# hkust-vgd/scanobjectnn

Measured on NVIDIA H100. Metric: point-clouds/sec (B=32, N=2048, 15-class), higher is better.
Workload: dtype f32

## Files before the change

### scanobjectnn_b200/csrc/tc_mlp.cu

```cuda
#include <float.h>
#include <stdlib.h>

#include <algorithm>
#include <atomic>
#include <type_traits>

#include "common.cuh"
#include "mlp_internal.cuh"
#include "ring_gemm.cuh"
#include "tc_common.cuh"

namespace psa {

using namespace tc;

constexpr int kMaxTcLayers = 2;


struct TcArgs {
    long long groups;
    int K;
    int n, m;
    const float* xyz;
    const float* new_xyz;
    const float* uf;
    const int* idx;
    float* out;
    const float* w1c;
    const float* w1x;
    const float* s1;
    const float* t1;
    int C1, relu1;
    int nl;
    const uint8_t* image[kMaxTcLayers];
    const float* s[kMaxTcLayers];
    const float* t[kMaxTcLayers];
    int relu[kMaxTcLayers];
    int Kd[kMaxTcLayers], Ntot[kMaxTcLayers];
    int stream_last;
    int joint;
    int pool_chunks;
    unsigned int* tile_counter;
    int np;
    unsigned int* ovf;
    const unsigned int* run_if;
    const unsigned int* wflag[kMaxTcLayers];
    const float* colscale[kMaxTcLayers];
};

template <int NP, int S>
__device__ __forceinline__ void put_a(uint32_t (&A)[NP][S][4], int s, int r, float x0, float x1, uint32_t& ovf) {
    uint32_t p[NP];
    split_pair<NP>(x0, x1, p, ovf);
#pragma unroll
    for (int i = 0; i < NP; ++i) A[i][s][r] = p[i];
}

__device__ __forceinline__ float warp_rowmax16(float lo, float hi) {
    float m = fmaxf(lo, hi);
    m = fmaxf(m, __shfl_xor_sync(0xffffffffu, m, 4));
    m = fmaxf(m, __shfl_xor_sync(0xffffffffu, m, 8));
    m = fmaxf(m, __shfl_xor_sync(0xffffffffu, m, 16));
    return m;
}
template <int H, int S>
__device__ __forceinline__ void colmax_halve(float (&v)[S], bool up) {
#pragma unroll
    for (int i = 0; i < H; ++i) {
        const float lo = v[i], hi = v[H + i];
        v[i] = fmaxf(up ? hi : lo, __shfl_xor_sync(0xffffffffu, up ? lo : hi, 2 * H));
    }
}
__device__ __forceinline__ float warp_rowsum16(float v) {
    v += __shfl_xor_sync(0xffffffffu, v, 4);
    v += __shfl_xor_sync(0xffffffffu, v, 8);
    v += __shfl_xor_sync(0xffffffffu, v, 16);
    return v;
}

__global__ void __launch_bounds__(256) tc_col_scale_kernel(int K, int N, const float* __restrict__ W, float* __restrict__ colscale,
                                                           unsigned int* __restrict__ trailer) {
    __shared__ float s_max[8][32];
    __shared__ int s_bad[8][32];
    const int n = blockIdx.x * 32 + threadIdx.x;
    float m = 0.f;
    bool bad = false;
    if (n < N)
        for (int k = threadIdx.y; k < K; k += 8) {
            const float w = __ldg(W + (size_t)k * N + n);
            bad = bad || !isfinite(w);
            m = fmaxf(m, fabsf(w));
        }
    s_max[threadIdx.y][threadIdx.x] = m;
    s_bad[threadIdx.y][threadIdx.x] = bad;
    __syncthreads();
    if (threadIdx.y != 0 || n >= N) return;
    for (int y = 1; y < 8; ++y) { m = fmaxf(m, s_max[y][threadIdx.x]); bad = bad || s_bad[y][threadIdx.x]; }
    int e = 0;
    if (!bad && m > 0.f) e = min(137 - (int)(__float_as_uint(m) >> 23), 64);
    colscale[n] = __int_as_float((127 - e) << 23);
    if (bad) atomicOr(trailer, 1u);
}

template <int NP>
__global__ void tc_prep_weights_kernel(int K, int Kp, int N, int Nt, const float* __restrict__ W, const float* __restrict__ colscale,
                                       uint8_t* __restrict__ image, const unsigned int* __restrict__ run_if) {
    if (run_if != nullptr && *run_if == 0u) return;
    const int KC = Kp / 64;
    const uint32_t bb = tc_block_bytes(Nt, NP), piece = (uint32_t)Nt * 128u;
    uint32_t unused = 0u;
    for (int e = blockIdx.x * blockDim.x + threadIdx.x; e < Kp * N; e += gridDim.x * blockDim.x) {
        const int n = e % N, k = e / N;
        float w = k < K ? __ldg(W + e) : 0.f;
        if (NP == 2) w *= pow2_rcp(__ldg(colscale + n));
        uint32_t pc[NP];
        split_pair<NP>(w, 0.f, pc, unused);
        uint8_t* blk = image + (size_t)((n / Nt) * KC + (k >> 6)) * bb;
        const uint32_t off = swz_off_bf16(n % Nt, k & 63, Nt);
#pragma unroll
        for (int i = 0; i < NP; ++i) *reinterpret_cast<uint16_t*>(blk + i * piece + off) = (uint16_t)(pc[i] & 0xffffu);
    }
}

constexpr int kSaNt = 64;
constexpr int kSaThreads = 256;
constexpr uint32_t kSmemBudget = 220u * 1024u;

struct TcSaLayout {
    uint32_t w[kMaxTcLayers];
    uint32_t ring[2];
    uint32_t ring_bytes;
    uint32_t vec, total;
};

__host__ __device__ inline TcSaLayout tc_sa_layout(const TcArgs& a) {
    TcSaLayout L;
    uint32_t off = 0;
#pragma unroll
    for (int l = 0; l < kMaxTcLayers; ++l) {
        L.w[l] = off;
        if (l < a.nl && !(a.stream_last && l == a.nl - 1)) off += (uint32_t)tc_image_bytes(a.Kd[l], a.Ntot[l], a.np);
    }
    L.ring_bytes = a.stream_last ? (uint32_t)(a.Kd[a.nl - 1] / 64) * tc_block_bytes(kSaNt, a.np) : 0u;
    L.ring[0] = off; off += L.ring_bytes;
    L.ring[1] = off; off += L.ring_bytes;
    L.vec = off;
    off += 7u * a.C1 * 4u;
#pragma unroll
    for (int l = 0; l < kMaxTcLayers; ++l) off += l < a.nl ? 2u * a.Ntot[l] * 4u : 0u;
    L.total = off;
    return L;
}

__host__ __device__ inline int sa_chunk(int K, bool joint) { return (joint ? 128 : 512) / K; }
__host__ __device__ inline uint32_t sa_carry_bytes(const TcArgs& a) { return a.joint ? 0u : 2u * a.Ntot[a.nl - 1] * 4u; }
__host__ __device__ inline uint32_t sa_red_bytes(int chunks) { return 8u * 64u * 4u * (uint32_t)chunks; }

__device__ __forceinline__ void sa_fill_ring(uint32_t q, const uint8_t* image, int ncl, const TcSaLayout& L, uint8_t* base, uint64_t* bars) {
    uint64_t* bar = &bars[q & 1];
    mbar_expect_tx(bar, L.ring_bytes);
    const uint8_t* src = image + (size_t)(q % (uint32_t)ncl) * L.ring_bytes;
    for (uint32_t o = 0; o < L.ring_bytes; o += 32768u) bulk_g2s(base + L.ring[q & 1] + o, src + o, min(32768u, L.ring_bytes - o), bar);
}

template <int NP, int KS, int NCH>
__device__ __forceinline__ void sa_mma_issue(float (&d)[NCH][32], const uint32_t (&A)[NP][8][4], uint32_t wb, uint32_t cstride) {
    constexpr uint32_t bb = tc_block_bytes(kSaNt, NP), piece = kSaNt * 128u;
    wg_fence();
#pragma unroll
    for (int tt = 0; tt < Split<NP>::kTerms; ++tt)
#pragma unroll
        for (int s = 0; s < KS; ++s)
#pragma unroll
            for (int c = 0; c < NCH; ++c)
                wg_mma_rs<NP>(d[c], A[Split<NP>::a(tt)][s][0], A[Split<NP>::a(tt)][s][1], A[Split<NP>::a(tt)][s][2], A[Split<NP>::a(tt)][s][3],
                              wg_desc(wb + (uint32_t)c * cstride + (uint32_t)(s >> 2) * bb + Split<NP>::w(tt) * piece + (uint32_t)(s & 3) * 32u),
                              (tt | s) ? 1u : 0u);
    wg_commit();
}
template <int NP, int KS, int NCH>
__device__ __forceinline__ void sa_mma(float (&d)[NCH][32], const uint32_t (&A)[NP][8][4], uint32_t wb, uint32_t cstride) {
    sa_mma_issue<NP, KS, NCH>(d, A, wb, cstride);
    wg_wait_all();
#pragma unroll
    for (int c = 0; c < NCH; ++c) wg_fence_acc(d[c]);
}

#ifdef PSA_SA_STAMPS
enum SaStamp { kSaTop, kSaInputs, kSaLayer1, kSaL2Issued, kSaL2Retired, kSaL2Epi, kSaPool1, kSaPool2, kSaNextA, kSaNextB, kSaChunk0 };
constexpr int kSaStampCtas = 264, kSaStampPasses = 64, kSaStampPhases = kSaChunk0 + 3 * 4;
__device__ long long g_sa_stamps[kSaStampCtas][2][kSaStampPasses][kSaStampPhases];
extern "C" PSA_API int psa_sa_stamps(long long* dst) {
    return cudaMemcpyFromSymbol(dst, g_sa_stamps, sizeof(g_sa_stamps)) == cudaSuccess ? 0 : 1;
}
extern "C" PSA_API int psa_sa_stamps_clear(void) {
    void* p = nullptr;
    if (cudaGetSymbolAddress(&p, g_sa_stamps) != cudaSuccess) return 1;
    return cudaMemset(p, 0, sizeof(g_sa_stamps)) == cudaSuccess ? 0 : 1;
}
#define SA_STAMP(p, k)                                                                                              \
    do {                                                                                                            \
        if ((threadIdx.x & 127) == 0 && blockIdx.x < kSaStampCtas && (p) < kSaStampPasses && (k) < kSaStampPhases) \
            g_sa_stamps[blockIdx.x][threadIdx.x >> 7][(p)][(k)] = clock64();                                        \
    } while (0)
#define SA_STAMP_AFTER(p, k, r)                                                                                     \
    do {                                                                                                            \
        if ((threadIdx.x & 127) == 0 && blockIdx.x < kSaStampCtas && (p) < kSaStampPasses) {                        \
            volatile long long* p_ = &g_sa_stamps[blockIdx.x][threadIdx.x >> 7][(p)][(k)];                          \
            *p_ = (long long)__float_as_uint(__fmul_rn((r), 0.f));                                                  \
            *p_ = clock64();                                                                                        \
        }                                                                                                           \
    } while (0)
#else
#define SA_STAMP(p, k) \
    do {               \
    } while (0)
#define SA_STAMP_AFTER(p, k, r) \
    do {                        \
    } while (0)
#endif

template <int NP, int C1, int NL, int N0>
__global__ void __launch_bounds__(kSaThreads, NP == 2 && C1 == 64 && (NL == 1 || N0 == 64) ? 2 : 1)
tc_sa_kernel(const __grid_constant__ TcArgs a) {
    static_assert((C1 == 64 || C1 == 128) && (NL == 1 || (NL == 2 && (N0 == 64 || N0 == 128))), "unsupported level shape");
    constexpr int last = NL - 1;
    constexpr int KSL = (NL == 2 ? N0 : C1) / 16;
    constexpr bool kDouble = !(C1 == 64 && (NL == 1 || N0 == 64));
    if (a.run_if != nullptr && *a.run_if == 0u) return;
    constexpr uint32_t bb = tc_block_bytes(kSaNt, NP);
    uint32_t ovf = 0u;
    bool ovf_seen = false;
    extern __shared__ uint8_t smem_raw[];
    __shared__ __align__(8) uint64_t s_rbar;
    __shared__ __align__(8) uint64_t s_wbar[2];
    __shared__ unsigned int s_claim[2];
    __shared__ int s_slots[2][2][16];
    __shared__ long long s_desc[2][2][8];

    const int tid = threadIdx.x, lane = tid & 31, warp = tid >> 5;
    const int g = lane >> 2, t = lane & 3;
    uint8_t* base = smem_raw + ((1024u - (smem_u32(smem_raw) & 1023u)) & 1023u);
    const TcSaLayout L = tc_sa_layout(a);

    float* vec = reinterpret_cast<float*>(base + L.vec);
    float* w1x = vec;
    float* w1c = vec + 3 * C1;
    float* t1 = vec + 6 * C1;
    float* sl0 = t1 + C1;
    float* tl0 = sl0 + a.Ntot[0];
    float* slL = NL == 2 ? tl0 + a.Ntot[0] : sl0;
    float* tlL = slL + a.Ntot[last];
    for (int i = tid; i < 3 * C1; i += kSaThreads) {
        const float sc = a.s1 ? __ldg(a.s1 + i % C1) : 1.f;
        w1x[i] = __ldg(a.w1x + i) * sc;
        w1c[i] = (a.w1c ? __ldg(a.w1c + i) : 0.f) * sc - (a.uf ? w1x[i] : 0.f);
    }
    for (int i = tid; i < C1; i += kSaThreads) t1[i] = __ldg(a.t1 + i);
#pragma unroll
    for (int l = 0; l < NL; ++l)
        for (int i = tid; i < a.Ntot[l]; i += kSaThreads) {
            (l == 0 ? sl0 : slL)[i] = (a.s[l] ? __ldg(a.s[l] + i) : 1.f) * (NP == 2 ? __ldg(a.colscale[l] + i) : 1.f);
            (l == 0 ? tl0 : tlL)[i] = __ldg(a.t[l] + i);
        }
    if (tid == 0) {
        mbar_init(&s_rbar, 1); mbar_init(&s_wbar[0], 1); mbar_init(&s_wbar[1], 1);
        fence_mbar_init();
    }
    __syncthreads();

    const int NCL = a.Ntot[last] / 64;
    uint32_t resident = 0;
#pragma unroll
    for (int l = 0; l < NL; ++l)
        if (!(a.stream_last && l == last)) resident += (uint32_t)tc_image_bytes(a.Kd[l], a.Ntot[l], NP);
    if (tid == 0) {
        if (resident) {
            mbar_expect_tx(&s_rbar, resident);
#pragma unroll
            for (int l = 0; l < NL; ++l) {
                if (a.stream_last && l == last) continue;
                const uint32_t bytes = (uint32_t)tc_image_bytes(a.Kd[l], a.Ntot[l], NP);
                for (uint32_t o = 0; o < bytes; o += 32768u) bulk_g2s(base + L.w[l] + o, a.image[l] + o, min(32768u, bytes - o), &s_rbar);
            }
        }
        if (a.stream_last) { sa_fill_ring(0, a.image[last], NCL, L, base, s_wbar); sa_fill_ring(1, a.image[last], NCL, L, base, s_wbar); }
    }
    if (resident) mbar_wait(&s_rbar, 0);

    const int K = a.K;
    const bool joint = a.joint;
    const int W = joint ? 8 : 4;
    const int C = sa_chunk(K, joint);
    const int unit = joint ? 0 : warp >> 2;
    const int ubar = 1 + unit, uthreads = 32 * W;
    const int ut = joint ? tid : tid & 127, uw0 = joint ? 0 : 4 * unit;
    const int wl = warp - uw0;
    const unsigned nchunks = (unsigned)((a.groups + C - 1) / C);
    float* carry = reinterpret_cast<float*>(base + L.total) + (size_t)unit * a.Ntot[last];
    const int NG = a.pool_chunks, rs = 64 * NG;
    float* red = reinterpret_cast<float*>(base + L.total + sa_carry_bytes(a)) + (size_t)warp * rs;

    auto fill_table = [&](unsigned ch, int b) {
        const long long g0 = (long long)ch * C;
        if (joint) {
            if (ut < C) s_slots[unit][b][ut] = g0 + ut < a.groups ? K / 16 : 0;
            return;
        }
        const long long r0 = g0 * K + wl * 128, rows = a.groups * K;
        int v[4];
#pragma unroll
        for (int q = 0; q < 4; ++q) v[q] = r0 + 32 * q + lane < rows ? __ldg(a.idx + r0 + 32 * q + lane) : 0;
        if (K == 32) {
#pragma unroll
            for (int q = 0; q < 4; ++q) {
                const unsigned d = __ballot_sync(0xffffffffu, v[q] != __shfl_sync(0xffffffffu, v[q], 0));
                const int nb = 4 * wl + q, Ln = d ? 32 - __clz(d) : 1;
                if (lane == 0) s_slots[unit][b][nb] = g0 + nb < a.groups ? (Ln + 15) >> 4 : 0;
            }
        } else {
#pragma unroll
            for (int h = 0; h < 2; ++h) {
                const int f = __shfl_sync(0xffffffffu, v[2 * h], 0);
                const unsigned lo = __ballot_sync(0xffffffffu, v[2 * h] != f), hi = __ballot_sync(0xffffffffu, v[2 * h + 1] != f);
                const int nb = 2 * wl + h, Ln = hi ? 64 - __clz(hi) : lo ? 32 - __clz(lo) : 1;
                if (lane == 0) s_slots[unit][b][nb] = g0 + nb < a.groups ? (Ln + 15) >> 4 : 0;
            }
        }
    };

    constexpr bool kAhead = NL == 2;
    constexpr bool kHoldU = NP == 2 && C1 == 128 && kAhead;
    constexpr int kUH = kHoldU ? C1 / 8 : 1;
    int incl = 0;
    int jn[2];
    long long gn = 0;
    bool carry_next = false;
    float cx = 0.f, cy = 0.f, cz = 0.f, px[2], py[2], pz[2];
    const float* urow[2];
    float2 uh[2][kUH];
    auto gather_a = [&](unsigned ch, int b, int p, int d) {
        if (p == 0) {
            incl = lane < C ? s_slots[unit][b][lane] : 0;
#pragma unroll
            for (int o = 1; o < 16; o <<= 1) {
                const int y = __shfl_up_sync(0xffffffffu, incl, o);
                if (lane >= o) incl += y;
            }
        }
        const int T = __shfl_sync(0xffffffffu, incl, C - 1);
        const int s = p * W + wl, ss = min(s, T - 1);
        const int nb = __popc(__ballot_sync(0xffffffffu, incl <= ss) & ((1u << C) - 1u));
        const int end = __shfl_sync(0xffffffffu, incl, nb), start = nb ? __shfl_sync(0xffffffffu, incl, nb - 1) : 0;
        gn = (long long)ch * C + nb;
        const int row = 16 * (ss - start) + g;
#pragma unroll
        for (int i = 0; i < 2; ++i) jn[i] = __ldg(a.idx + gn * K + row + 8 * i);
        const float* c = a.new_xyz + (size_t)gn * 3;
        cx = __ldg(c); cy = __ldg(c + 1); cz = __ldg(c + 2);
        carry_next = wl == 0 && s < T && s > start;
        if (lane == 0) {
            long long run = 0;
            if (s < T && (wl == 0 || s == start)) {
                const int pe = (p + 1) * W;
                run = gn << 8 | (long long)(min(end, pe) - s) | (s > start ? 16 : 0) | (end > pe ? 32 : 0);
            }
            s_desc[unit][d][wl] = run;
        }
    };
    auto gather_b = [&]() {
        const long long bi = gn / a.m;
#pragma unroll
        for (int i = 0; i < 2; ++i) {
            if (a.uf == nullptr) {
                const float* p = a.xyz + ((size_t)bi * a.n + jn[i]) * 3;
                px[i] = __ldg(p); py[i] = __ldg(p + 1); pz[i] = __ldg(p + 2);
            }
            urow[i] = a.uf ? a.uf + ((size_t)bi * a.n + jn[i]) * C1 : nullptr;
            if constexpr (kHoldU) {
                if (a.uf != nullptr) {
#pragma unroll
                    for (int q = 0; q < kUH; ++q) uh[i][q] = __ldg(reinterpret_cast<const float2*>(urow[i] + 8 * q + 2 * t));
                }
            }
        }
    };

    if (ut == 0) s_claim[unit] = atomicAdd(a.tile_counter, 1u);
    unit_bar_sync(ubar, uthreads);
    unsigned ch = s_claim[unit], claimed = 0;
    if (ch < nchunks) fill_table(ch, 0);
    unit_bar_sync(ubar, uthreads);
    int buf = 0, p = 0;
    if (kAhead && ch < nchunks) { gather_a(ch, 0, 0, 0); gather_b(); }
    uint32_t it = 0;
    for (; ch < nchunks; ++it) {
        if (p == 0 && ut == 0) s_claim[unit] = atomicAdd(a.tile_counter, 1u);
        SA_STAMP(it, kSaTop);
        if (!kAhead) { gather_a(ch, buf, p, it & 1); gather_b(); }
        SA_STAMP_AFTER(it, kSaInputs, a.uf == nullptr ? px[0] : kHoldU ? uh[0][0].x : __ldg(urow[0] + 2 * t));

        uint32_t A[NP][8][4];
        if (a.uf != nullptr) {
#pragma unroll
            for (int s = 0; s < C1 / 16; ++s) {
#pragma unroll
                for (int h = 0; h < 2; ++h) {
                    const int k = 16 * s + 8 * h + 2 * t;
                    const float2 cwx = *reinterpret_cast<const float2*>(w1c + k), cwy = *reinterpret_cast<const float2*>(w1c + C1 + k),
                                 cwz = *reinterpret_cast<const float2*>(w1c + 2 * C1 + k);
                    const float2 ct = ffma2_rn(make_float2(cz, cz), cwz, ffma2_rn(make_float2(cy, cy), cwy, fmul2_rn(make_float2(cx, cx), cwx)));
#pragma unroll
                    for (int i = 0; i < 2; ++i) {
                        float2 v;
                        if constexpr (kHoldU) v = uh[i][2 * s + h];
                        else v = __ldg(reinterpret_cast<const float2*>(urow[i] + k));
                        v = fadd2_rn(v, ct);
                        if (a.relu1) { v.x = fmaxf(v.x, 0.f); v.y = fmaxf(v.y, 0.f); }
                        put_a<NP, 8>(A, s, i + 2 * h, v.x, v.y, ovf);
                    }
                }
            }
        } else {
            float dx[2], dy[2], dz[2];
#pragma unroll
            for (int i = 0; i < 2; ++i) { dx[i] = px[i] - cx; dy[i] = py[i] - cy; dz[i] = pz[i] - cz; }
#pragma unroll
            for (int s = 0; s < C1 / 16; ++s) {
#pragma unroll
                for (int h = 0; h < 2; ++h) {
                    const int k = 16 * s + 8 * h + 2 * t;
                    const float2 sh = *reinterpret_cast<const float2*>(t1 + k);
                    const float2 wx = *reinterpret_cast<const float2*>(w1x + k), wy = *reinterpret_cast<const float2*>(w1x + C1 + k),
                                 wz = *reinterpret_cast<const float2*>(w1x + 2 * C1 + k);
#pragma unroll
                    for (int i = 0; i < 2; ++i) {
                        float2 v = sh;
                        if (a.w1c != nullptr) {
                            const float2 cwx = *reinterpret_cast<const float2*>(w1c + k), cwy = *reinterpret_cast<const float2*>(w1c + C1 + k),
                                         cwz = *reinterpret_cast<const float2*>(w1c + 2 * C1 + k);
                            v = ffma2_rn(make_float2(cz, cz), cwz, ffma2_rn(make_float2(cy, cy), cwy, ffma2_rn(make_float2(cx, cx), cwx, v)));
                        }
                        v = ffma2_rn(make_float2(dz[i], dz[i]), wz, ffma2_rn(make_float2(dy[i], dy[i]), wy, ffma2_rn(make_float2(dx[i], dx[i]), wx, v)));
                        if (a.relu1) { v.x = fmaxf(v.x, 0.f); v.y = fmaxf(v.y, 0.f); }
                        put_a<NP, 8>(A, s, i + 2 * h, v.x, v.y, ovf);
                    }
                }
            }
        }
        SA_STAMP(it, kSaLayer1);

        if constexpr (NL == 2) {
            constexpr int NCH = N0 / 64;
            float d[NCH][32];
            sa_mma_issue<NP, C1 / 16, NCH>(d, A, smem_u32(base + L.w[0]), (uint32_t)(C1 / 64) * bb);
            SA_STAMP(it, kSaL2Issued);
            wg_wait_all();
#pragma unroll
            for (int c = 0; c < NCH; ++c) wg_fence_acc(d[c]);
            SA_STAMP(it, kSaL2Retired);
#pragma unroll
            for (int c = 0; c < NCH; ++c) {
#pragma unroll
                for (int jj = 0; jj < 4; ++jj) {
#pragma unroll
                    for (int h = 0; h < 2; ++h) {
                        const int j = 2 * jj + h, col = c * 64 + 8 * j + 2 * t;
                        const float sc0 = sl0[col], sc1 = sl0[col + 1], sh0 = tl0[col], sh1 = tl0[col + 1];
#pragma unroll
                        for (int i = 0; i < 2; ++i) {
                            float v0 = fmaf(d[c][4 * j + 2 * i], sc0, sh0), v1 = fmaf(d[c][4 * j + 2 * i + 1], sc1, sh1);
                            if (a.relu[0]) { v0 = fmaxf(v0, 0.f); v1 = fmaxf(v1, 0.f); }
                            put_a<NP, 8>(A, c * 4 + jj, i + 2 * h, v0, v1, ovf);
                        }
                    }
                }
            }
            SA_STAMP(it, kSaL2Epi);
        }
        if constexpr (NP == 2) { ovf_seen = ovf_seen || f16x2_overflowed(ovf); ovf = 0u; }
        {
            const int N = a.Ntot[last];
            const bool carry_in = carry_next;
            const bool same = (p + 1) * W < __shfl_sync(0xffffffffu, incl, C - 1);
            const bool ahead = kAhead && (same || (p > 0 && claimed < nchunks));
            const bool after_pool = kAhead && !same && p == 0;
            auto issue = [&](float (&acc)[1][32], int nc) {
                uint32_t wb;
                if (a.stream_last) {
                    const uint32_t q = it * (uint32_t)NCL + (uint32_t)nc;
                    mbar_wait(&s_wbar[q & 1], (q >> 1) & 1u);
                    wb = smem_u32(base + L.ring[q & 1]);
                } else {
                    wb = smem_u32(base + L.w[last]) + (uint32_t)(nc * (KSL / 4)) * bb;
                }
                sa_mma_issue<NP, KSL, 1>(acc, A, wb, 0u);
                SA_STAMP(it, kSaChunk0 + 3 * nc);
            };
            auto epilogue = [&](float (&acc)[1][32], int nc) {
                wg_fence_acc(acc[0]);
                SA_STAMP(it, kSaChunk0 + 3 * nc + 1);
                auto rowmax = [&](int j) {
                    const int col = nc * 64 + 8 * j + 2 * t;
                    const float2 sc = *reinterpret_cast<const float2*>(slL + col), sh = *reinterpret_cast<const float2*>(tlL + col);
                    float lo0 = fmaf(acc[0][4 * j], sc.x, sh.x), hi0 = fmaf(acc[0][4 * j + 2], sc.x, sh.x);
                    float lo1 = fmaf(acc[0][4 * j + 1], sc.y, sh.y), hi1 = fmaf(acc[0][4 * j + 3], sc.y, sh.y);
                    if (a.relu[last]) { lo0 = fmaxf(lo0, 0.f); hi0 = fmaxf(hi0, 0.f); lo1 = fmaxf(lo1, 0.f); hi1 = fmaxf(hi1, 0.f); }
                    return make_float2(fmaxf(lo0, hi0), fmaxf(lo1, hi1));
                };
                float v[8];
                const bool up = (g >> 2) & 1;
#pragma unroll
                for (int j = 0; j < 4; ++j) {
                    const float2 lo = rowmax(j), hi = rowmax(j + 4);
                    v[2 * j] = fmaxf(up ? hi.x : lo.x, __shfl_xor_sync(0xffffffffu, up ? lo.x : hi.x, 16));
                    v[2 * j + 1] = fmaxf(up ? hi.y : lo.y, __shfl_xor_sync(0xffffffffu, up ? lo.y : hi.y, 16));
                }
                colmax_halve<4>(v, (g >> 1) & 1);
                colmax_halve<2>(v, g & 1);
                float2 m = make_float2(v[0], v[1]);
                const int x = 8 * g + 2 * t;
                float* dst = red + (nc % NG) * 64 + x;
                {
                    const float2 c = *reinterpret_cast<const float2*>(carry_in ? carry + nc * 64 + x : dst);
                    m.x = carry_in ? fmaxf(m.x, c.x) : m.x;
                    m.y = carry_in ? fmaxf(m.y, c.y) : m.y;
                }
                *reinterpret_cast<float2*>(dst) = m;
                SA_STAMP(it, kSaChunk0 + 3 * nc + 2);
            };
            auto pool = [&](int gi) {
                unit_bar_sync(ubar, uthreads);
                SA_STAMP(it, kSaPool1);
                if (gi == 0 && p == 0) {
                    claimed = s_claim[unit];
                    if (claimed < nchunks) fill_table(claimed, buf ^ 1);
                }
                if (a.stream_last && tid == 0)
                    sa_fill_ring(it * (uint32_t)NCL + (uint32_t)gi + 2u, a.image[last], NCL, L, base, s_wbar);
                const long long run = s_desc[unit][it & 1][wl];
                const int len = (int)(run & 15);
                if (len != 0) {
                    for (int c = 0; c < NG; ++c) {
                        const float2* r = reinterpret_cast<const float2*>(red + c * 64) + lane;
                        float2 mx = r[0];
#pragma unroll
                        for (int w = 1; w < 8; ++w)
                            if (w < len) { const float2 v = r[w * rs / 2]; mx.x = fmaxf(mx.x, v.x); mx.y = fmaxf(mx.y, v.y); }
                        const int col = (gi * NG + c) * 64 + 2 * lane;
                        if (run & 32) *reinterpret_cast<float2*>(carry + col) = mx;
                        else *reinterpret_cast<float2*>(a.out + (size_t)(run >> 8) * N + col) = mx;
                    }
                }
                unit_bar_sync(ubar, uthreads);
                SA_STAMP(it, kSaPool2);
                if (gi == 0 && after_pool && claimed < nchunks) {
                    gather_a(claimed, buf ^ 1, 0, (it + 1) & 1);
                    SA_STAMP(it, kSaNextA);
                    gather_b();
                    SA_STAMP(it, kSaNextB);
                }
            };
            float d0[1][32];
            for (int c0 = 0; c0 < NCL; c0 += NG) {
                const int end = c0 + NG;
                issue(d0, c0);
                if (ahead && c0 == 0) {
                    gather_a(same ? ch : claimed, same ? buf : buf ^ 1, same ? p + 1 : 0, (it + 1) & 1);
                    SA_STAMP(it, kSaNextA);
                }
                if constexpr (kDouble) {
                    float d1[1][32];
                    int nc = c0;
                    for (; nc + 2 < end; nc += 2) {
                        issue(d1, nc + 1); wg_wait<1>(); epilogue(d0, nc);
                        issue(d0, nc + 2); wg_wait<1>(); epilogue(d1, nc + 1);
                    }
                    if (nc + 1 < end) {
                        issue(d1, nc + 1); wg_wait<1>(); epilogue(d0, nc);
                        if (ahead && nc + 2 == NCL) { gather_b(); SA_STAMP(it, kSaNextB); }
                        wg_wait<0>(); epilogue(d1, nc + 1);
                    } else {
                        if (ahead && nc + 1 == NCL) { gather_b(); SA_STAMP(it, kSaNextB); }
                        wg_wait<0>(); epilogue(d0, nc);
                    }
                } else {
                    for (int nc = c0;;) {
                        if (ahead && nc + 1 == NCL) { gather_b(); SA_STAMP(it, kSaNextB); }
                        wg_wait<0>(); epilogue(d0, nc);
                        if (++nc == end) break;
                        issue(d0, nc);
                    }
                }
                pool(c0 / NG);
            }
            if (!same) { ch = claimed; buf ^= 1; p = 0; }
            else ++p;
        }
    }
    if constexpr (NP == 2) {
        if (ovf_seen) atomicOr(a.ovf, 1u);
        if (tid == 0)
            for (int l = 0; l < NL; ++l)
                if (a.wflag[l] != nullptr && *a.wflag[l] != 0u) atomicOr(a.ovf, 1u);
    }
    if (tid == 0 && a.stream_last)
        for (uint32_t q = it * (uint32_t)NCL; q < it * (uint32_t)NCL + 2u; ++q) mbar_wait(&s_wbar[q & 1], (q >> 1) & 1u);
}

struct TcDenseArgs {
    long long rows;
    int K, Kp, N;
    int pool_k;
    int relu;
    const float* x;
    const float* scale;
    const float* shift;
    const float* xyz3;
    const float* w3;
    float* out;
    const float* in_scale = nullptr;
    const float* in_shift = nullptr;
    int in_relu = 0;
    float* stat_partial = nullptr;
    const float* group_add = nullptr;
    long long group_rows = 0;
    RingArgs ring;
};

template <int NP, int NC>
struct DenseOp {
    static constexpr int Nt = 64 * NC;
    const TcDenseArgs& a;
    static constexpr bool kClaim = true;
    static constexpr uint32_t kBudget = 210u * 1024u;
    struct Smem {
        float red[2][8][Nt];
        __align__(16) float aff[2][3][Nt];
    };
    struct Unit {
        int nb, col0, par;
        long long tile;
        long long r[2];
        bool v[2];
    };

    __device__ int units(int) const { return (int)((a.rows + 127) / 128 * (a.N / Nt)); }

    template <class Put>
    __device__ void produce(int unit, int, int pw, int lane, Smem&, Put&& put) const {
        const int NTC = a.N / Nt, KC = a.Kp / 64;
        const long long row0 = (long long)(unit / NTC) * 128;
        const int nt = unit % NTC, r0 = 32 * pw, nr = (int)max(0LL, min(32LL, a.rows - row0 - r0));
        if ((a.K & 3) == 0 && (reinterpret_cast<uintptr_t>(a.x) & 15) == 0) {
            for (int kb = 0; kb < KC; ++kb) put((size_t)nt * KC + kb, [&](uint32_t xs) { stage_rows16(xs, a.x, a.K, row0, r0, nr, kb, a.K, lane); });
            return;
        }
        for (int kb = 0; kb < KC; ++kb)
            put((size_t)nt * KC + kb, [&](uint32_t xs) {
#pragma unroll 1
                for (int e = lane; e < nr * 64; e += 32) {
                    const int row = r0 + (e >> 6), c = e & 63;
                    if (kb * 64 + c < a.K) cp_async4(xs + (uint32_t)row * kRingXRow + (uint32_t)c * 4u, a.x + (size_t)(row0 + row) * a.K + kb * 64 + c);
                }
            });
    }

    __device__ Unit unit(int unit, int, int row, Smem& sm, int n) const {
        const int NTC = a.N / Nt, tid = threadIdx.x;
        Unit u;
        u.nb = a.Kp / 64;
        u.tile = unit / NTC;
        u.col0 = unit % NTC * Nt;
        u.par = n & 1;
#pragma unroll
        for (int i = 0; i < 2; ++i) {
            u.r[i] = u.tile * 128 + row + 8 * i;
            u.v[i] = u.r[i] < a.rows;
        }
        if (tid < Nt) {
            const int col = u.col0 + tid;
            const float cs = NP == 2 ? __ldg(a.ring.colscale + col) : 1.f;
            sm.aff[u.par][0][tid] = (a.scale ? __ldg(a.scale + col) : 1.f) * cs;
            sm.aff[u.par][1][tid] = a.shift ? __ldg(a.shift + col) : 0.f;
// ... 236 lines not shown
    d.x = s.x; d.W = s.W; d.scale = s.scale; d.shift = s.shift; d.out = s.out;
    d.group_add = s.group_add; d.group_rows = s.group_rows; d.xyz3 = s.xyz3; d.w3 = s.w3;
    if (s.fc_partial != nullptr && s.rows <= 32 && s.pool_k == 1 && s.group_add == nullptr && s.xyz3 == nullptr) return launch_fc_small(d, s.fc_partial, st);
    return launch_dense(d, st);
}

bool tc_train_fwd_eligible(long long rows, int K, int N) {
    return rows >= 128 && K >= 128 && K <= 512 && N >= 128 && (N % 128) == 0;
}
int launch_tc_dense_train(long long rows, int K, int N, const float* x, const float* in_scale, const float* in_shift, int in_relu,
                          const float* W, const float* bias, float* y, float* stat_partial, uint8_t* image_ws, cudaStream_t st) {
    const int Kp = (K + 63) & ~63;
    int rc = build_image(K, Kp, N, 128 | kImageBf16x3, W, image_ws, st);
    if (rc != PSA_OK) return rc;
    TcDenseArgs a;
    a.rows = rows; a.K = K; a.Kp = Kp; a.N = N; a.pool_k = 1; a.relu = 0;
    a.x = x; a.scale = nullptr; a.shift = bias; a.out = y; a.xyz3 = nullptr; a.w3 = nullptr;
    a.in_scale = in_scale; a.in_shift = in_shift; a.in_relu = in_relu; a.stat_partial = stat_partial;
    a.ring.image = image_ws;
    return ring_launch(kDenseRing, 3, 128, &a, tc_dense_units(rows, N, 128), st);
}

static const uint8_t* prebuilt_image(const psa_mlp* mlp, int l, int row0, int Nt) {
    if (mlp->image[l] != nullptr && mlp->image_nt[l] == Nt && mlp->image_row0[l] == row0) return reinterpret_cast<const uint8_t*>(mlp->image[l]);
    return nullptr;
}

bool tc_sa_eligible(const psa_mlp* mlp, int c, int nsample, TcArgs* out, int np) {
    if (mlp->n_layers < 2 || mlp->n_layers > 1 + kMaxTcLayers) return false;
    if (!(nsample == 32 || nsample == 64 || nsample == 128)) return false;
    if (mlp->channels[0] != 3 + c) return false;
    const int C1 = mlp->channels[1];
    if (!(C1 == 64 || C1 == 128)) return false;
    TcArgs a{};
    a.C1 = C1;
    a.nl = mlp->n_layers - 1;
    a.np = np;
    for (int l = 0; l < a.nl; ++l) {
        a.Kd[l] = mlp->channels[1 + l];
        a.Ntot[l] = mlp->channels[2 + l];
        if (!(a.Kd[l] == 64 || a.Kd[l] == 128)) return false;
        const bool is_last = (l == a.nl - 1);
        if (!is_last && !(a.Ntot[l] == 64 || a.Ntot[l] == 128)) return false;
        if (is_last && !(a.Ntot[l] == 64 || a.Ntot[l] % 128 == 0)) return false;
    }
    a.stream_last = 0;
    if (tc_sa_layout(a).total + 1024 > kSmemBudget) a.stream_last = 1;
    if (tc_sa_layout(a).total + 1024 > kSmemBudget) return false;
    *out = a;
    return true;
}
bool tc_sa_eligible(const psa_mlp* mlp, int c, int nsample, TcArgs* out) {
    TcArgs a3;
    if (!tc_sa_eligible(mlp, c, nsample, &a3, 3)) return false;
    if (g_tc_np == 3) { *out = a3; return true; }
    return tc_sa_eligible(mlp, c, nsample, out, 2);
}

size_t tc_sa_workspace_bytes(const TcArgs& a, int b, int n, int c) {
    size_t bytes = 256;
    for (int l = 0; l < a.nl; ++l) bytes += tc_image_alloc_bytes(a.Kd[l], a.Ntot[l], 2) + tc_image_alloc_bytes(a.Kd[l], a.Ntot[l], 3);
    if (c > 0) bytes += (((size_t)b * n * a.C1 * sizeof(float) + 255) & ~(size_t)255) + tc_dense_image_bytes(c, a.C1);
    return bytes;
}

static int tc_sa_image_nt() { return kSaNt | image_flag(g_tc_np); }

template <int NP, int C1, int NL, int N0>
static int launch_tc_sa_shape(const TcArgs& a, long long ctas_needed, size_t smem, cudaStream_t st) {
    PSA_CUDA(cudaFuncSetAttribute(tc_sa_kernel<NP, C1, NL, N0>, cudaFuncAttributeMaxDynamicSharedMemorySize, (int)smem));
    int dev = 0, sms = 0, per_sm = 0;
    PSA_CUDA(cudaGetDevice(&dev));
    PSA_CUDA(cudaDeviceGetAttribute(&sms, cudaDevAttrMultiProcessorCount, dev));
    PSA_CUDA(cudaOccupancyMaxActiveBlocksPerMultiprocessor(&per_sm, tc_sa_kernel<NP, C1, NL, N0>, kSaThreads, smem));
    const long long resident = (long long)sms * (per_sm > 0 ? per_sm : 1);
    const int ctas = (int)(ctas_needed < 1 ? 1 : ctas_needed < resident ? ctas_needed : resident);
    tc_sa_kernel<NP, C1, NL, N0><<<ctas, kSaThreads, smem, st>>>(a);
    return check_launch("tc_sa_kernel");
}

template <int NP>
static int launch_tc_sa_np(TcArgs& a, cudaStream_t st) {
    const uint32_t limit = 223u * 1024u;
    a.joint = a.K == 128 || a.stream_last;
    if (!a.joint && tc_sa_layout(a).total + 1024 + sa_carry_bytes(a) + sa_red_bytes(1) > limit) a.joint = 1;
    const size_t used = (size_t)tc_sa_layout(a).total + 1024 + sa_carry_bytes(a);
    const int ncl = a.Ntot[a.nl - 1] / 64;
    a.pool_chunks = 1;
    if (!a.stream_last)
        for (int ng = ncl; ng > 1; --ng)
            if (ncl % ng == 0 && used + sa_red_bytes(ng) <= limit) { a.pool_chunks = ng; break; }
    const int C = sa_chunk(a.K, a.joint);
    const long long nchunks = (a.groups + C - 1) / C;
    const long long ctas_needed = a.joint ? nchunks : (nchunks + 1) / 2;
    const size_t smem = used + sa_red_bytes(a.pool_chunks);
    if (a.nl == 1) return a.C1 == 64 ? launch_tc_sa_shape<NP, 64, 1, 0>(a, ctas_needed, smem, st) : launch_tc_sa_shape<NP, 128, 1, 0>(a, ctas_needed, smem, st);
    if (a.C1 == 64) return a.Ntot[0] == 64 ? launch_tc_sa_shape<NP, 64, 2, 64>(a, ctas_needed, smem, st) : launch_tc_sa_shape<NP, 64, 2, 128>(a, ctas_needed, smem, st);
    return a.Ntot[0] == 64 ? launch_tc_sa_shape<NP, 128, 2, 64>(a, ctas_needed, smem, st) : launch_tc_sa_shape<NP, 128, 2, 128>(a, ctas_needed, smem, st);
}

static int tc_sa_run(TcArgs& a, int b, int n, int m, int c, int nsample, const float* xyz, const float* new_xyz, const float* points,
                     const int* idx, const psa_mlp* mlp, const float* w1c, float* out, void* workspace, cudaStream_t st) {
    int rc = PSA_OK;
    uint8_t* ws = reinterpret_cast<uint8_t*>(workspace);
    unsigned int* region = reinterpret_cast<unsigned int*>(ws);
    const StepWords words = step_words(region, 1);
    PSA_CUDA(cudaMemsetAsync(ws, 0, 256, st));
    ws += 256;
    RingWeights w[kMaxTcLayers];
    for (int l = 0; l < a.nl; ++l) {
        const int K = a.Kd[l], N = a.Ntot[l];
        w[l] = RingWeights{K, K, N, kSaNt, mlp->weight[1 + l], ws, ws + tc_image_alloc_bytes(K, N, 2), prebuilt_image(mlp, 1 + l, 0, tc_sa_image_nt())};
        ws += tc_image_alloc_bytes(K, N, 2) + tc_image_alloc_bytes(K, N, 3);
    }
    const float* uf = nullptr;
    if (c > 0) {
        const long long rows = (long long)b * n;
        DenseStep u{rows, c, a.C1, 1, 0, points, mlp->weight[0] + (size_t)3 * a.C1, mlp->scale[0], mlp->shift[0], reinterpret_cast<float*>(ws)};
        u.xyz3 = xyz;
        u.w3 = mlp->weight[0];
        u.prebuilt = prebuilt_image(mlp, 0, 3, tc_dense_nt(rows, a.C1));
        u.img = ws + (((size_t)rows * a.C1 * sizeof(float) + 255) & ~(size_t)255);
        u.words = step_words(region, 0);
        if ((rc = run_dense(u, st)) != PSA_OK) return rc;
        uf = u.out;
    }
    auto fill = [&](TcArgs& t) {
        t.groups = (long long)b * m; t.K = nsample; t.n = n; t.m = m;
        t.xyz = xyz; t.new_xyz = new_xyz; t.idx = idx; t.out = out; t.uf = uf;
        t.w1x = mlp->weight[0]; t.s1 = mlp->scale[0]; t.t1 = mlp->shift[0]; t.relu1 = mlp->relu[0];
        t.ovf = nullptr; t.run_if = nullptr; t.w1c = w1c;
        for (int l = 0; l < t.nl; ++l) {
            t.s[l] = mlp->scale[1 + l]; t.t[l] = mlp->shift[1 + l]; t.relu[l] = mlp->relu[1 + l]; t.wflag[l] = nullptr; t.colscale[l] = nullptr;
        }
    };
    fill(a);
    for (int l = 0; l < a.nl; ++l) {
        if ((rc = ring_image(w[l], a.np, nullptr, st, a.image[l])) != PSA_OK) return rc;
        if (a.np == 2) { a.wflag[l] = image_trailer(a.image[l], w[l].Kp, w[l].N); a.colscale[l] = image_colscale(a.image[l], w[l].Kp, w[l].N); }
    }
    a.tile_counter = words.counters;
    if (a.np == 3) return launch_tc_sa_np<3>(a, st);
    a.ovf = words.flag;
    rc = launch_tc_sa_np<2>(a, st);
    if (rc != PSA_OK) return rc;
    TcArgs a3;
    PSA_REQUIRE(tc_sa_eligible(mlp, c, nsample, &a3, 3), "sa_module: internal error (bf16x3 eligibility)");
    fill(a3);
    for (int l = 0; l < a3.nl; ++l)
        if ((rc = ring_image(w[l], 3, words.flag, st, a3.image[l])) != PSA_OK) return rc;
    a3.tile_counter = words.counters + 1;
    a3.run_if = words.flag;
    return launch_tc_sa_np<3>(a3, st);
}

struct TcGroupAllArgs {
    int c;
    int N[3];
    int Nt[3];
    const float* points;
    const float* xyz;
    const float* w3;
    const uint8_t* image[3];
    const float* colscale[3];
    const unsigned int* wflag[3];
    const float* scale[3];
    const float* shift[3];
    int relu[3];
    float* out;
    unsigned int* ovf;
};

constexpr int kGaStages = 3;
constexpr uint32_t kGaStageBytes = 32768u;
constexpr uint32_t kGaSmemBudget = 222u * 1024u;
constexpr uint32_t kGaSliceBytes = 32768u;
__device__ __forceinline__ uint32_t ga_frag_off(int warp, int lane, int q) { return (uint32_t)(((warp * 8 + q) * 32 + lane) * 16); }
__host__ __device__ inline uint32_t group_all_smem(int W0, int W1, int W2) {
// ... 683 lines not shown
```

Baseline: 98580.

## Replace per-warp reduction and carry pooling with shared-memory atomic max buffers

Max-pooling over neighbour rows changes from per-warp partial buffers, run descriptors and carry state to a per-chunk shared-memory pool. Warps fold their column maxima into it with red.shared.max on order-preserving integer codes, and the pool is flushed to global memory once per chunk, so the per-pass pool barriers and reduction loops are gone. The chunk claim is double-buffered, overflow flags are reported immediately, and stream_last is forced when the pool does not fit in shared memory. The risks are atomic contention on shared memory, the extra per-chunk store and reset pass, and a larger shared-memory footprint that may lower occupancy.

After: 103,300, median of 6. 4.8% higher.

```diff
diff --git a/scanobjectnn_b200/csrc/tc_mlp.cu b/scanobjectnn_b200/csrc/tc_mlp.cu
--- a/scanobjectnn_b200/csrc/tc_mlp.cu
+++ b/scanobjectnn_b200/csrc/tc_mlp.cu
@@ -39,7 +39,6 @@
     int Kd[kMaxTcLayers], Ntot[kMaxTcLayers];
     int stream_last;
     int joint;
-    int pool_chunks;
     unsigned int* tile_counter;
     int np;
     unsigned int* ovf;
@@ -153,8 +152,17 @@
 }
 
 __host__ __device__ inline int sa_chunk(int K, bool joint) { return (joint ? 128 : 512) / K; }
-__host__ __device__ inline uint32_t sa_carry_bytes(const TcArgs& a) { return a.joint ? 0u : 2u * a.Ntot[a.nl - 1] * 4u; }
-__host__ __device__ inline uint32_t sa_red_bytes(int chunks) { return 8u * 64u * 4u * (uint32_t)chunks; }
+__host__ __device__ inline int sa_pool_cols(const TcArgs& a) { return a.stream_last ? 64 : a.Ntot[a.nl - 1]; }
+__host__ __device__ inline uint32_t sa_pool_bytes(const TcArgs& a) {
+    return (a.joint ? 1u : 2u) * (uint32_t)sa_chunk(a.K, a.joint) * (uint32_t)sa_pool_cols(a) * 4u;
+}
+__device__ __forceinline__ int sa_pool_code(float x) {
+    const int b = __float_as_int(x);
+    return b >= 0 ? b : b ^ 0x7fffffff;
+}
+__device__ __forceinline__ float sa_pool_value(int c) { return __int_as_float(c >= 0 ? c : c ^ 0x7fffffff); }
+__device__ __forceinline__ void red_smem_max(uint32_t addr, int v) { asm volatile("red.shared.max.s32 [%0], %1;\n" ::"r"(addr), "r"(v) : "memory"); }
+constexpr int kSaPoolEmpty = (int)0x807fffff;
 
 __device__ __forceinline__ void sa_fill_ring(uint32_t q, const uint8_t* image, int ncl, const TcSaLayout& L, uint8_t* base, uint64_t* bars) {
     uint64_t* bar = &bars[q & 1];
@@ -187,7 +195,7 @@
 }
 
 #ifdef PSA_SA_STAMPS
-enum SaStamp { kSaTop, kSaInputs, kSaLayer1, kSaL2Issued, kSaL2Retired, kSaL2Epi, kSaPool1, kSaPool2, kSaNextA, kSaNextB, kSaChunk0 };
+enum SaStamp { kSaTop, kSaInputs, kSaLayer1, kSaL2Issued, kSaL2Retired, kSaL2Epi, kSaEnd1, kSaEnd2, kSaNextA, kSaNextB, kSaChunk0 };
 constexpr int kSaStampCtas = 264, kSaStampPasses = 64, kSaStampPhases = kSaChunk0 + 3 * 4;
 __device__ long long g_sa_stamps[kSaStampCtas][2][kSaStampPasses][kSaStampPhases];
 extern "C" PSA_API int psa_sa_stamps(long long* dst) {
@@ -230,13 +238,11 @@
     if (a.run_if != nullptr && *a.run_if == 0u) return;
     constexpr uint32_t bb = tc_block_bytes(kSaNt, NP);
     uint32_t ovf = 0u;
-    bool ovf_seen = false;
     extern __shared__ uint8_t smem_raw[];
     __shared__ __align__(8) uint64_t s_rbar;
     __shared__ __align__(8) uint64_t s_wbar[2];
-    __shared__ unsigned int s_claim[2];
+    __shared__ unsigned int s_chunk[2][2];
     __shared__ int s_slots[2][2][16];
-    __shared__ long long s_desc[2][2][8];
 
     const int tid = threadIdx.x, lane = tid & 31, warp = tid >> 5;
     const int g = lane >> 2, t = lane & 3;
@@ -263,6 +269,7 @@
             (l == 0 ? sl0 : slL)[i] = (a.s[l] ? __ldg(a.s[l] + i) : 1.f) * (NP == 2 ? __ldg(a.colscale[l] + i) : 1.f);
             (l == 0 ? tl0 : tlL)[i] = __ldg(a.t[l] + i);
         }
+    for (uint32_t i = tid; i < sa_pool_bytes(a) / 4u; i += kSaThreads) reinterpret_cast<int*>(base + L.total)[i] = kSaPoolEmpty;
     if (tid == 0) {
         mbar_init(&s_rbar, 1); mbar_init(&s_wbar[0], 1); mbar_init(&s_wbar[1], 1);
         fence_mbar_init();
@@ -297,9 +304,8 @@
     const int ut = joint ? tid : tid & 127, uw0 = joint ? 0 : 4 * unit;
     const int wl = warp - uw0;
     const unsigned nchunks = (unsigned)((a.groups + C - 1) / C);
-    float* carry = reinterpret_cast<float*>(base + L.total) + (size_t)unit * a.Ntot[last];
-    const int NG = a.pool_chunks, rs = 64 * NG;
-    float* red = reinterpret_cast<float*>(base + L.total + sa_carry_bytes(a)) + (size_t)warp * rs;
+    const int PC = sa_pool_cols(a);
+    const uint32_t pool = L.total + (uint32_t)(unit * C * PC) * 4u;
 
     auto fill_table = [&](unsigned ch, int b) {
         const long long g0 = (long long)ch * C;
@@ -335,11 +341,12 @@
     int incl = 0;
     int jn[2];
     long long gn = 0;
-    bool carry_next = false;
     float cx = 0.f, cy = 0.f, cz = 0.f, px[2], py[2], pz[2];
     const float* urow[2];
     float2 uh[2][kUH];
-    auto gather_a = [&](unsigned ch, int b, int p, int d) {
+    auto slot_total = [&]() { return __shfl_sync(0xffffffffu, incl, C - 1); };
+    auto slot_nb = [&](int p) { return __popc(__ballot_sync(0xffffffffu, incl <= min(p * W + wl, slot_total() - 1)) & ((1u << C) - 1u)); };
+    auto gather_a = [&](unsigned ch, int b, int p) {
         if (p == 0) {
             incl = lane < C ? s_slots[unit][b][lane] : 0;
 #pragma unroll
@@ -348,25 +355,14 @@
                 if (lane >= o) incl += y;
             }
         }
-        const int T = __shfl_sync(0xffffffffu, incl, C - 1);
-        const int s = p * W + wl, ss = min(s, T - 1);
-        const int nb = __popc(__ballot_sync(0xffffffffu, incl <= ss) & ((1u << C) - 1u));
-        const int end = __shfl_sync(0xffffffffu, incl, nb), start = nb ? __shfl_sync(0xffffffffu, incl, nb - 1) : 0;
+        const int ss = min(p * W + wl, slot_total() - 1), nb = slot_nb(p);
+        const int start = nb ? __shfl_sync(0xffffffffu, incl, nb - 1) : 0;
         gn = (long long)ch * C + nb;
         const int row = 16 * (ss - start) + g;
 #pragma unroll
         for (int i = 0; i < 2; ++i) jn[i] = __ldg(a.idx + gn * K + row + 8 * i);
         const float* c = a.new_xyz + (size_t)gn * 3;
         cx = __ldg(c); cy = __ldg(c + 1); cz = __ldg(c + 2);
-        carry_next = wl == 0 && s < T && s > start;
-        if (lane == 0) {
-            long long run = 0;
-            if (s < T && (wl == 0 || s == start)) {
-                const int pe = (p + 1) * W;
-                run = gn << 8 | (long long)(min(end, pe) - s) | (s > start ? 16 : 0) | (end > pe ? 32 : 0);
-            }
-            s_desc[unit][d][wl] = run;
-        }
     };
     auto gather_b = [&]() {
         const long long bi = gn / a.m;
@@ -374,7 +370,8 @@
         for (int i = 0; i < 2; ++i) {
             if (a.uf == nullptr) {
                 const float* p = a.xyz + ((size_t)bi * a.n + jn[i]) * 3;
-                px[i] = __ldg(p); py[i] = __ldg(p + 1); pz[i] = __ldg(p + 2);
+                if constexpr (kHoldU) { uh[i][0] = make_float2(__ldg(p), __ldg(p + 1)); uh[i][1].x = __ldg(p + 2); }
+                else { px[i] = __ldg(p); py[i] = __ldg(p + 1); pz[i] = __ldg(p + 2); }
             }
             urow[i] = a.uf ? a.uf + ((size_t)bi * a.n + jn[i]) * C1 : nullptr;
             if constexpr (kHoldU) {
@@ -386,19 +383,18 @@
         }
     };
 
-    if (ut == 0) s_claim[unit] = atomicAdd(a.tile_counter, 1u);
+    if (ut == 0) s_chunk[unit][0] = atomicAdd(a.tile_counter, 1u);
     unit_bar_sync(ubar, uthreads);
-    unsigned ch = s_claim[unit], claimed = 0;
-    if (ch < nchunks) fill_table(ch, 0);
+    if (s_chunk[unit][0] < nchunks) fill_table(s_chunk[unit][0], 0);
     unit_bar_sync(ubar, uthreads);
     int buf = 0, p = 0;
-    if (kAhead && ch < nchunks) { gather_a(ch, 0, 0, 0); gather_b(); }
+    if (kAhead && s_chunk[unit][0] < nchunks) { gather_a(s_chunk[unit][0], 0, 0); gather_b(); }
     uint32_t it = 0;
-    for (; ch < nchunks; ++it) {
-        if (p == 0 && ut == 0) s_claim[unit] = atomicAdd(a.tile_counter, 1u);
+    for (; s_chunk[unit][buf] < nchunks; ++it) {
+        if (p == 0 && ut == 0) s_chunk[unit][buf ^ 1] = atomicAdd(a.tile_counter, 1u);
         SA_STAMP(it, kSaTop);
-        if (!kAhead) { gather_a(ch, buf, p, it & 1); gather_b(); }
-        SA_STAMP_AFTER(it, kSaInputs, a.uf == nullptr ? px[0] : kHoldU ? uh[0][0].x : __ldg(urow[0] + 2 * t));
+        if (!kAhead) { gather_a(s_chunk[unit][buf], buf, p); gather_b(); }
+        SA_STAMP_AFTER(it, kSaInputs, kHoldU ? uh[0][0].x : a.uf == nullptr ? px[0] : __ldg(urow[0] + 2 * t));
 
         uint32_t A[NP][8][4];
         if (a.uf != nullptr) {
@@ -424,7 +420,10 @@
         } else {
             float dx[2], dy[2], dz[2];
 #pragma unroll
-            for (int i = 0; i < 2; ++i) { dx[i] = px[i] - cx; dy[i] = py[i] - cy; dz[i] = pz[i] - cz; }
+            for (int i = 0; i < 2; ++i) {
+                if constexpr (kHoldU) { dx[i] = uh[i][0].x - cx; dy[i] = uh[i][0].y - cy; dz[i] = uh[i][1].x - cz; }
+                else { dx[i] = px[i] - cx; dy[i] = py[i] - cy; dz[i] = pz[i] - cz; }
+            }
 #pragma unroll
             for (int s = 0; s < C1 / 16; ++s) {
 #pragma unroll
@@ -478,13 +477,15 @@
             }
             SA_STAMP(it, kSaL2Epi);
         }
-        if constexpr (NP == 2) { ovf_seen = ovf_seen || f16x2_overflowed(ovf); ovf = 0u; }
+        if constexpr (NP == 2) {
+            if (f16x2_overflowed(ovf)) atomicOr(a.ovf, 1u);
+            ovf = 0u;
+        }
         {
             const int N = a.Ntot[last];
-            const bool carry_in = carry_next;
-            const bool same = (p + 1) * W < __shfl_sync(0xffffffffu, incl, C - 1);
-            const bool ahead = kAhead && (same || (p > 0 && claimed < nchunks));
-            const bool after_pool = kAhead && !same && p == 0;
+            const int NG = a.stream_last ? 1 : NCL;
+            const bool same = (p + 1) * W < slot_total();
+            const bool ahead = kAhead && same;
             auto issue = [&](float (&acc)[1][32], int nc) {
                 uint32_t wb;
                 if (a.stream_last) {
@@ -518,44 +519,34 @@
                 }
                 colmax_halve<4>(v, (g >> 1) & 1);
                 colmax_halve<2>(v, g & 1);
-                float2 m = make_float2(v[0], v[1]);
-                const int x = 8 * g + 2 * t;
-                float* dst = red + (nc % NG) * 64 + x;
-                {
-                    const float2 c = *reinterpret_cast<const float2*>(carry_in ? carry + nc * 64 + x : dst);
-                    m.x = carry_in ? fmaxf(m.x, c.x) : m.x;
-                    m.y = carry_in ? fmaxf(m.y, c.y) : m.y;
-                }
-                *reinterpret_cast<float2*>(dst) = m;
+                const uint32_t dst = smem_u32(base + pool) + 4u * (uint32_t)(slot_nb(p) * PC + (a.stream_last ? 0 : nc * 64) + 8 * g + 2 * t);
+                red_smem_max(dst, sa_pool_code(v[0]));
+                red_smem_max(dst + 4u, sa_pool_code(v[1]));
                 SA_STAMP(it, kSaChunk0 + 3 * nc + 2);
             };
-            auto pool = [&](int gi) {
+            auto store = [&](int c0) {
                 unit_bar_sync(ubar, uthreads);
-                SA_STAMP(it, kSaPool1);
-                if (gi == 0 && p == 0) {
-                    claimed = s_claim[unit];
-                    if (claimed < nchunks) fill_table(claimed, buf ^ 1);
-                }
+                SA_STAMP(it, kSaEnd1);
+                const unsigned next = s_chunk[unit][buf ^ 1];
+                const bool last_store = c0 + NG == NCL;
+                if (last_store && next < nchunks) fill_table(next, buf ^ 1);
                 if (a.stream_last && tid == 0)
-                    sa_fill_ring(it * (uint32_t)NCL + (uint32_t)gi + 2u, a.image[last], NCL, L, base, s_wbar);
-                const long long run = s_desc[unit][it & 1][wl];
-                const int len = (int)(run & 15);
-                if (len != 0) {
-                    for (int c = 0; c < NG; ++c) {
-                        const float2* r = reinterpret_cast<const float2*>(red + c * 64) + lane;
-                        float2 mx = r[0];
-#pragma unroll
-                        for (int w = 1; w < 8; ++w)
-                            if (w < len) { const float2 v = r[w * rs / 2]; mx.x = fmaxf(mx.x, v.x); mx.y = fmaxf(mx.y, v.y); }
-                        const int col = (gi * NG + c) * 64 + 2 * lane;
-                        if (run & 32) *reinterpret_cast<float2*>(carry + col) = mx;
-                        else *reinterpret_cast<float2*>(a.out + (size_t)(run >> 8) * N + col) = mx;
+                    sa_fill_ring(it * (uint32_t)NCL + (uint32_t)c0 + 2u, a.image[last], NCL, L, base, s_wbar);
+                const long long g0 = (long long)s_chunk[unit][buf] * C;
+                const int rows = (int)min((long long)C, a.groups - g0), half = PC / 2;
+                for (int e = ut; e < C * half; e += uthreads) {
+                    int2* const q = reinterpret_cast<int2*>(base + pool) + e;
+                    const int r = e / half, col = c0 * 64 + 2 * (e - r * half);
+                    if (r < rows) {
+                        const int2 c = *q;
+                        *reinterpret_cast<float2*>(a.out + (size_t)(g0 + r) * N + col) = make_float2(sa_pool_value(c.x), sa_pool_value(c.y));
                     }
+                    *q = make_int2(kSaPoolEmpty, kSaPoolEmpty);
                 }
                 unit_bar_sync(ubar, uthreads);
-                SA_STAMP(it, kSaPool2);
-                if (gi == 0 && after_pool && claimed < nchunks) {
-                    gather_a(claimed, buf ^ 1, 0, (it + 1) & 1);
+                SA_STAMP(it, kSaEnd2);
+                if (kAhead && last_store && next < nchunks) {
+                    gather_a(next, buf ^ 1, 0);
                     SA_STAMP(it, kSaNextA);
                     gather_b();
                     SA_STAMP(it, kSaNextB);
@@ -566,7 +557,7 @@
                 const int end = c0 + NG;
                 issue(d0, c0);
                 if (ahead && c0 == 0) {
-                    gather_a(same ? ch : claimed, same ? buf : buf ^ 1, same ? p + 1 : 0, (it + 1) & 1);
+                    gather_a(s_chunk[unit][buf], buf, p + 1);
                     SA_STAMP(it, kSaNextA);
                 }
                 if constexpr (kDouble) {
@@ -592,14 +583,13 @@
                         issue(d0, nc);
                     }
                 }
-                pool(c0 / NG);
-            }
-            if (!same) { ch = claimed; buf ^= 1; p = 0; }
+                if (!same) store(c0);
+            }
+            if (!same) { buf ^= 1; p = 0; }
             else ++p;
         }
     }
     if constexpr (NP == 2) {
-        if (ovf_seen) atomicOr(a.ovf, 1u);
         if (tid == 0)
             for (int l = 0; l < NL; ++l)
                 if (a.wflag[l] != nullptr && *a.wflag[l] != 0u) atomicOr(a.ovf, 1u);
@@ -1002,18 +992,15 @@
 template <int NP>
 static int launch_tc_sa_np(TcArgs& a, cudaStream_t st) {
     const uint32_t limit = 223u * 1024u;
+    auto fits = [&] { return tc_sa_layout(a).total + 1024u + sa_pool_bytes(a) <= limit; };
     a.joint = a.K == 128 || a.stream_last;
-    if (!a.joint && tc_sa_layout(a).total + 1024 + sa_carry_bytes(a) + sa_red_bytes(1) > limit) a.joint = 1;
-    const size_t used = (size_t)tc_sa_layout(a).total + 1024 + sa_carry_bytes(a);
-    const int ncl = a.Ntot[a.nl - 1] / 64;
-    a.pool_chunks = 1;
-    if (!a.stream_last)
-        for (int ng = ncl; ng > 1; --ng)
-            if (ncl % ng == 0 && used + sa_red_bytes(ng) <= limit) { a.pool_chunks = ng; break; }
+    if (!a.joint && !fits()) a.joint = 1;
+    if (!fits()) a.stream_last = 1;
+    PSA_REQUIRE(fits(), "sa_module: internal error (pooling buffer does not fit)");
     const int C = sa_chunk(a.K, a.joint);
     const long long nchunks = (a.groups + C - 1) / C;
     const long long ctas_needed = a.joint ? nchunks : (nchunks + 1) / 2;
-    const size_t smem = used + sa_red_bytes(a.pool_chunks);
+    const size_t smem = (size_t)tc_sa_layout(a).total + 1024 + sa_pool_bytes(a);
     if (a.nl == 1) return a.C1 == 64 ? launch_tc_sa_shape<NP, 64, 1, 0>(a, ctas_needed, smem, st) : launch_tc_sa_shape<NP, 128, 1, 0>(a, ctas_needed, smem, st);
     if (a.C1 == 64) return a.Ntot[0] == 64 ? launch_tc_sa_shape<NP, 64, 2, 64>(a, ctas_needed, smem, st) : launch_tc_sa_shape<NP, 64, 2, 128>(a, ctas_needed, smem, st);
     return a.Ntot[0] == 64 ? launch_tc_sa_shape<NP, 128, 2, 64>(a, ctas_needed, smem, st) : launch_tc_sa_shape<NP, 128, 2, 128>(a, ctas_needed, smem, st);
```
